# jinkyu032/TPDM

Measured on NVIDIA B200. Metric: images/sec/box, SD3-M 1024^2 TPDM sampling, higher is better.
Workload: dtype bf16

## Files before the change

tpdm_b200/csrc/gemm2_tcgen05.cu:

```cuda
#include <cuda_bf16.h>

#include "common.cuh"
#include "gemm_epilogue.cuh"
#include "host.h"

namespace tpdm {

namespace {

constexpr int BM = 128;
constexpr int BN2 = 256;
#ifndef TPDM_GEMM2_BK
#define TPDM_GEMM2_BK 64
#endif
constexpr int BK = TPDM_GEMM2_BK;
constexpr int kSub = BK / 64;
constexpr int kStages2 = BK == 64 ? 5 : 3;
constexpr int kEpiWarps2 = 8;
constexpr int kThreads2 = 64 + 32 * kEpiWarps2;
constexpr int kABytes2 = BM * BK * 2;
constexpr int kBBytes2 = (BN2 / 2) * BK * 2;
constexpr int kStageBytes2 = kABytes2 + kBBytes2;
constexpr int kRing2 = kStages2 * kStageBytes2;
constexpr int kEpi2 = kEpiWarps2 * 32 * kStagePad * 4 + kEpiWarps2 * 2 * (BN2 / 2) * 4;
constexpr int kBarOff2 = kRing2 + kEpi2;
constexpr int kSmem2 = kBarOff2 + 256 + 1024;

#ifdef TPDM_GEMM_TRACE
__device__ long long g_gemm_trace[4096];
__device__ int g_gemm_trace_n;
#endif

struct Gemm2Params {
  GemmOp op[2];
  int n_ops;
  int tiles0, total_tiles;
  const int* skip;
  const int* bmask;
  int bslots;
};

struct PairCoord {
  int g, b, mtp, nt;
};

__device__ __forceinline__ PairCoord decode_pair(const Gemm2Params& P, int tile) {
  PairCoord t;
  t.g = (P.n_ops > 1 && tile >= P.tiles0) ? 1 : 0;
  const int local = tile - (t.g ? P.tiles0 : 0);
  const GemmOp& G = P.op[t.g];
  const int tiles_mp = (G.rows_per_batch + 2 * BM - 1) / (2 * BM);
  const int m_idx = local / G.tiles_n;
  t.nt = local - m_idx * G.tiles_n;
  t.b = m_idx / tiles_mp;
  t.mtp = m_idx - t.b * tiles_mp;
  return t;
}

__device__ __forceinline__ uint32_t cluster_ctarank() {
  uint32_t r;
  asm volatile("mov.u32 %0, %%cluster_ctarank;" : "=r"(r));
  return r;
}
__device__ __forceinline__ void cluster_sync_all() {
  asm volatile("barrier.cluster.arrive.release.aligned;\n\tbarrier.cluster.wait.acquire.aligned;\n" ::: "memory");
}
__device__ __forceinline__ uint32_t map_to_cta(const void* p, uint32_t rank) {
  uint32_t r;
  asm volatile("mapa.shared::cluster.u32 %0, %1, %2;" : "=r"(r) : "r"(smem_u32(p)), "r"(rank));
  return r;
}
__device__ __forceinline__ void mbar_arrive_expect_tx_cluster(uint32_t cluster_addr, uint32_t bytes) {
  asm volatile("mbarrier.arrive.expect_tx.shared::cluster.b64 _, [%0], %1;" ::"r"(cluster_addr), "r"(bytes) : "memory");
}
__device__ __forceinline__ void mbar_arrive_cluster(uint32_t cluster_addr) {
  asm volatile("mbarrier.arrive.shared::cluster.b64 _, [%0];" ::"r"(cluster_addr) : "memory");
}
__device__ __forceinline__ void tma2_load_3d(void* smem_dst, const CUtensorMap* m, uint32_t bar_cluster_addr, int c0, int c1, int c2) {
  asm volatile(
      "cp.async.bulk.tensor.3d.cta_group::2.shared::cluster.global.mbarrier::complete_tx::bytes [%0], [%1, {%3, %4, %5}], [%2];\n" ::"r"(
          smem_u32(smem_dst)),
      "l"(reinterpret_cast<uint64_t>(m)), "r"(bar_cluster_addr), "r"(c0), "r"(c1), "r"(c2)
      : "memory");
}
__device__ __forceinline__ void tma2_load_2d(void* smem_dst, const CUtensorMap* m, uint32_t bar_cluster_addr, int c0, int c1) {
  asm volatile(
      "cp.async.bulk.tensor.2d.cta_group::2.shared::cluster.global.mbarrier::complete_tx::bytes [%0], [%1, {%3, %4}], [%2];\n" ::"r"(
          smem_u32(smem_dst)),
      "l"(reinterpret_cast<uint64_t>(m)), "r"(bar_cluster_addr), "r"(c0), "r"(c1)
      : "memory");
}
__device__ __forceinline__ void umma2_ss(uint32_t d_tmem, uint64_t a_desc, uint64_t b_desc, uint32_t idesc, uint32_t accumulate) {
  asm volatile(
      "{\n\t.reg .pred p;\n\t"
      "setp.ne.b32 p, %4, 0;\n\t"
      "tcgen05.mma.cta_group::2.kind::f16 [%0], %1, %2, %3, p;\n\t}\n" ::"r"(d_tmem),
      "l"(a_desc), "l"(b_desc), "r"(idesc), "r"(accumulate)
      : "memory");
}
__device__ __forceinline__ void umma2_ss_elect(uint32_t d_tmem, uint64_t a_desc, uint64_t b_desc, uint32_t idesc, uint32_t accumulate) {
  asm volatile(
      "{\n\t.reg .pred p, e;\n\t"
      "elect.sync _|e, 0xffffffff;\n\t"
      "setp.ne.b32 p, %4, 0;\n\t"
      "@e tcgen05.mma.cta_group::2.kind::f16 [%0], %1, %2, %3, p;\n\t}\n" ::"r"(d_tmem),
      "l"(a_desc), "l"(b_desc), "r"(idesc), "r"(accumulate)
      : "memory");
}
__device__ __forceinline__ void umma2_commit_multicast_elect(uint64_t* bar) {
  asm volatile(
      "{\n\t.reg .pred e;\n\t"
      "elect.sync _|e, 0xffffffff;\n\t"
      "@e tcgen05.commit.cta_group::2.mbarrier::arrive::one.shared::cluster.multicast::cluster.b64 [%0], %1;\n\t}\n" ::"r"(smem_u32(bar)),
      "h"(static_cast<uint16_t>(3))
      : "memory");
}
__device__ __forceinline__ void umma2_commit_multicast(uint64_t* bar) {
  asm volatile("tcgen05.commit.cta_group::2.mbarrier::arrive::one.shared::cluster.multicast::cluster.b64 [%0], %1;\n" ::"r"(smem_u32(bar)),
               "h"(static_cast<uint16_t>(3))
               : "memory");
}

__global__ void __cluster_dims__(2, 1, 1) __launch_bounds__(kThreads2, 1) gemm2_bf16_tcgen05_kernel(const __grid_constant__ Gemm2Params P) {
  pdl_launch_dependents();
  extern __shared__ uint8_t smem_raw[];
  uint8_t* smem = reinterpret_cast<uint8_t*>((reinterpret_cast<uintptr_t>(smem_raw) + 1023) & ~uintptr_t(1023));
  float* epi_stage = reinterpret_cast<float*>(smem + kRing2);
  uint64_t* full_bar = reinterpret_cast<uint64_t*>(smem + kBarOff2);
  uint64_t* empty_bar = full_bar + kStages2;
  uint64_t* tmem_full = empty_bar + kStages2;
  uint64_t* tmem_empty = tmem_full + 2;
  uint32_t* tmem_slot = reinterpret_cast<uint32_t*>(tmem_empty + 2);

  const int warp = threadIdx.x >> 5;
  const int lane = threadIdx.x & 31;
  const uint32_t rank = cluster_ctarank();
  const int cluster_id = blockIdx.x >> 1, num_clusters = gridDim.x >> 1;

  if (warp == 0 && lane == 0) {
    for (int i = 0; i < P.n_ops; ++i) {
      tma_prefetch_desc(&P.op[i].tmA);
      tma_prefetch_desc(&P.op[i].tmB2);
    }
  }
  if (warp == 1 && lane == 0) {
    for (int i = 0; i < kStages2; ++i) {
      mbar_init(&full_bar[i], 2);
      mbar_init(&empty_bar[i], 1);
    }
    for (int i = 0; i < 2; ++i) {
      mbar_init(&tmem_full[i], 1);
      mbar_init(&tmem_empty[i], 2 * kEpiWarps2);
    }
    fence_barrier_init();
  }
  pdl_wait();
  if (P.skip != nullptr && *P.skip != 0) return;
  if (warp == 2) {
    asm volatile("tcgen05.alloc.cta_group::2.sync.aligned.shared::cta.b32 [%0], 512;\n" ::"r"(smem_u32(tmem_slot)) : "memory");
    asm volatile("tcgen05.relinquish_alloc_permit.cta_group::2.sync.aligned;\n" ::: "memory");
  }
  tc_fence_before();
  cluster_sync_all();
  tc_fence_after();
  const uint32_t tmem_base = *tmem_slot;

  if (warp == 0) {
    if (lane == 0) {
      int stage = 0;
      uint32_t phase = 0;
      for (int tile = cluster_id; tile < P.total_tiles; tile += num_clusters) {
        const PairCoord tc = decode_pair(P, tile);
        if (P.bmask != nullptr && P.bmask[tc.b % P.bslots] == 0) continue;
        const GemmOp& G = P.op[tc.g];
        const int nkb = (G.K + BK - 1) / BK;
        const int m0 = tc.mtp * 2 * BM + static_cast<int>(rank) * BM;
        const int nb0 = tc.nt * BN2 + static_cast<int>(rank) * (BN2 / 2);
        for (int kb = 0; kb < nkb; ++kb) {
          mbar_wait_backoff(&empty_bar[stage], phase ^ 1);
          uint8_t* sA = smem + stage * kStageBytes2;
          uint8_t* sB = sA + kABytes2;
          const uint32_t leader_full = map_to_cta(&full_bar[stage], 0);
          mbar_arrive_expect_tx_cluster(leader_full, kStageBytes2);
#pragma unroll
          for (int h = 0; h < kSub; ++h) {
            tma2_load_3d(sA + h * (BM * 128), &G.tmA, leader_full, kb * BK + h * 64, m0, tc.b);
            tma2_load_2d(sB + h * ((BN2 / 2) * 128), &G.tmB2, leader_full, kb * BK + h * 64, nb0);
          }
          if (++stage == kStages2) {
            stage = 0;
            phase ^= 1;
          }
        }
      }
    }
  } else if (warp == 1) {
    if (rank == 0) {
      constexpr uint32_t idesc = make_idesc_bf16(2 * BM, BN2);
      int stage = 0;
      uint32_t phase = 0;
      int acc = 0;
      uint32_t acc_phase = 0;
      for (int tile = cluster_id; tile < P.total_tiles; tile += num_clusters) {
        const PairCoord tc = decode_pair(P, tile);
        if (P.bmask != nullptr && P.bmask[tc.b % P.bslots] == 0) continue;
        const GemmOp& G = P.op[tc.g];
        const int nkb = (G.K + BK - 1) / BK;
#ifdef TPDM_GEMM_TRACE
        const bool tr = cluster_id == 0 && lane == 0;
        long long tq0 = 0;
        if (tr) tq0 = clock64();
#endif
        mbar_wait(&tmem_empty[acc], acc_phase ^ 1);
        tc_fence_after();
#ifdef TPDM_GEMM_TRACE
        if (tr && g_gemm_trace_n + 4 <= 4096) {
          g_gemm_trace[g_gemm_trace_n++] = -1;
          g_gemm_trace[g_gemm_trace_n++] = tq0;
          g_gemm_trace[g_gemm_trace_n++] = clock64();
          g_gemm_trace[g_gemm_trace_n++] = nkb;
        }
#endif
        const uint32_t d_tmem = tmem_base + acc * BN2;
        for (int kb = 0; kb < nkb; ++kb) {
#ifdef TPDM_GEMM_TRACE
          long long t0 = 0, t1 = 0;
          if (tr) t0 = clock64();
#endif
          mbar_wait(&full_bar[stage], phase);
          tc_fence_after();
#ifdef TPDM_GEMM_TRACE
          if (tr) t1 = clock64();
#endif
          {
            const uint32_t a_base = smem_u32(smem + stage * kStageBytes2);
            const uint32_t b_base = a_base + kABytes2;
            const uint64_t adesc0 = make_smem_desc_sw128(a_base, 16, 1024), bdesc0 = make_smem_desc_sw128(b_base, 16, 1024);
#pragma unroll
            for (int k = 0; k < BK / 16; ++k) {
              const uint32_t ao = ((k / 4) * (BM * 128) + (k % 4) * 32) >> 4, bo = ((k / 4) * ((BN2 / 2) * 128) + (k % 4) * 32) >> 4;
              umma2_ss_elect(d_tmem, adesc0 + ao, bdesc0 + bo, idesc, (kb | k) != 0 ? 1u : 0u);
            }
            umma2_commit_multicast_elect(&empty_bar[stage]);
            if (kb == nkb - 1) umma2_commit_multicast_elect(&tmem_full[acc]);
          }
#ifdef TPDM_GEMM_TRACE
          if (tr && g_gemm_trace_n + 3 <= 4096) {
            g_gemm_trace[g_gemm_trace_n++] = t0;
            g_gemm_trace[g_gemm_trace_n++] = t1;
            g_gemm_trace[g_gemm_trace_n++] = clock64();
          }
#endif
          __syncwarp();
          if (++stage == kStages2) {
            stage = 0;
            phase ^= 1;
          }
        }
        if (++acc == 2) {
          acc = 0;
          acc_phase ^= 1;
        }
      }
    }
  } else {
    const int q = warp & 3;
    const int hh = (warp - 2) >> 2;
    float* st = epi_stage + (warp - 2) * 32 * kStagePad;
    float* sbias = epi_stage + kEpiWarps2 * 32 * kStagePad + (warp - 2) * 2 * (BN2 / 2);
    int acc = 0;
    uint32_t acc_phase = 0;
    for (int tile = cluster_id; tile < P.total_tiles; tile += num_clusters) {
      const PairCoord tc = decode_pair(P, tile);
        if (P.bmask != nullptr && P.bmask[tc.b % P.bslots] == 0) continue;
      const GemmOp& G = P.op[tc.g];
      const int n0 = tc.nt * BN2;
      const int row_base = tc.mtp * 2 * BM + static_cast<int>(rank) * BM + q * 32;
      gemm_epilogue_tile<BN2>(
          G, tc.b, row_base, n0, tmem_base + (static_cast<uint32_t>(q * 32) << 16) + acc * BN2, st, sbias, lane, hh * (BN2 / 64), (hh + 1) * (BN2 / 64),
          [&]() { mbar_wait_backoff(&tmem_full[acc], acc_phase); },
          [&]() {
            if (lane == 0) mbar_arrive_cluster(map_to_cta(&tmem_empty[acc], 0));
          });
      if (++acc == 2) {
        acc = 0;
        acc_phase ^= 1;
      }
    }
  }

  __syncwarp();
  tc_fence_before();
  cluster_sync_all();
  if (warp == 2) asm volatile("tcgen05.dealloc.cta_group::2.sync.aligned.b32 %0, 512;\n" ::"r"(tmem_base) : "memory");
}

}

#ifdef TPDM_GEMM_TRACE
extern "C" int tpdm_gemm_trace_read(long long* host, int* n, int reset) {
  int cnt = 0;
  if (cudaMemcpyFromSymbol(&cnt, g_gemm_trace_n, sizeof(int)) != cudaSuccess) return -1;
  if (cudaMemcpyFromSymbol(host, g_gemm_trace, sizeof(long long) * 4096) != cudaSuccess) return -1;
  *n = cnt;
  if (reset) {
    cnt = 0;
    cudaMemcpyToSymbol(g_gemm_trace_n, &cnt, sizeof(int));
  }
  return 0;
}
#endif

int gemm2_launch(const GemmOp* ops, int n_ops, cudaStream_t stream) {
  TPDM_CHECK(n_ops >= 1 && n_ops <= 2, TPDM_ERR_ARG, "gemm2_launch: 1 or 2 ops per launch");
  Gemm2Params P;
  P.n_ops = n_ops;
  P.total_tiles = 0;
  P.tiles0 = 0;
  P.skip = skip_flag();
  P.bmask = batch_mask();
  P.bslots = batch_mask_slots();
  double flops = 0;
  for (int i = 0; i < n_ops; ++i) {
    TPDM_CHECK(ops[i].conv == 0 && ops[i].block_n == 256, TPDM_ERR_ARG, "gemm2_launch: plain GEMMs with 256-wide N tiles only");
    P.op[i] = ops[i];
    const int tiles_mp = (ops[i].rows_per_batch + 2 * BM - 1) / (2 * BM);
    const int t = ops[i].batch * tiles_mp * ops[i].tiles_n;
    if (i == 0) P.tiles0 = t;
    P.total_tiles += t;
    flops += 2.0 * ops[i].batch * ops[i].rows_per_batch * static_cast<double>(ops[i].N) * ops[i].K;
  }
  if (n_ops == 1) P.op[1] = ops[0];
  static bool attr_set = false;
  if (!attr_set) {
    TPDM_CUDA_OK(cudaFuncSetAttribute(gemm2_bf16_tcgen05_kernel, cudaFuncAttributeMaxDynamicSharedMemorySize, kSmem2));
    attr_set = true;
  }
  const int max_clusters = num_sms() / 2;
  const int clusters = P.total_tiles < max_clusters ? P.total_tiles : max_clusters;
  prof_begin(0, flops, stream);
  TPDM_CUDA_OK(launch_pdl(gemm2_bf16_tcgen05_kernel, dim3(2 * clusters), dim3(kThreads2), kSmem2, stream, P));
  prof_end(stream);
  count_launch();
  TPDM_CUDA_OK(cudaGetLastError());
  return 0;
}

}
```

tpdm_b200/csrc/gemm_epilogue.cuh:

```cuda
#pragma once
#include <cuda_bf16.h>

#include "common.cuh"
#include "host.h"

namespace tpdm {

constexpr int kStagePad = 36;

template <int BN, typename WaitFn, typename ReleaseFn>
__device__ __forceinline__ void gemm_epilogue_tile(const GemmOp& G, int batch_idx, int row_base, int n0, uint32_t tmem_acc, float* st,
                                                   float* sbias, int lane, int c_begin, int c_end, WaitFn wait_accumulator,
                                                   ReleaseFn release_accumulator) {
  int n_chunks = (G.N - n0 + 31) / 32;
  n_chunks = n_chunks > c_end ? c_end : n_chunks;
  const int ncol = (c_end - c_begin) * 32;
  if (n_chunks <= c_begin) {
    wait_accumulator();
    tc_fence_after();
    tc_fence_before();
    __syncwarp();
    release_accumulator();
    return;
  }
      int rows = G.rows_per_batch - row_base;
      rows = rows > 32 ? 32 : rows;
      const bool f32_out = G.epi == EPI_BIAS_F32 || G.epi == EPI_GATE_RESIDUAL;
      const bool add_bf16 = G.epi == EPI_BIAS_ADD_BF16;
      const bool resid = G.epi == EPI_GATE_RESIDUAL;
      const int vec = 4;
      const int cg = lane % 8;
      const int r_in = lane / 8;
      const float* gate_row = resid ? G.gate + static_cast<long long>(batch_idx) * G.gate_stride : nullptr;
      const long long tile_o0 = static_cast<long long>(batch_idx) * G.out_batch_stride + static_cast<long long>(row_base) * G.ldo + n0;

      auto load_resv = [&](int c, float4 (&rv)[8]) {
        const int col = n0 + c * 32 + cg * 4;
        if (col < G.N) {
          const float* o = reinterpret_cast<const float*>(G.out) + tile_o0 + c * 32 + cg * 4;
#pragma unroll
          for (int it = 0; it < 8; ++it) {
            const int r = it * 4 + r_in;
            rv[it] = r < rows ? *reinterpret_cast<const float4*>(o + static_cast<long long>(r) * G.ldo) : make_float4(0.f, 0.f, 0.f, 0.f);
          }
        }
      };
      for (int k = lane * 4; k < ncol; k += 128) {
        const int col = n0 + c_begin * 32 + k;
        float4 b4 = make_float4(0.f, 0.f, 0.f, 0.f), g4 = b4;
        if (col < G.N) {
          if (G.bias) b4 = *reinterpret_cast<const float4*>(G.bias + col);
          if (resid) g4 = *reinterpret_cast<const float4*>(gate_row + col);
        }
        *reinterpret_cast<float4*>(sbias + k) = b4;
        *reinterpret_cast<float4*>(sbias + ncol + k) = g4;
      }
      __syncwarp();
      float4 resv_a[8], resv_b[8];
      if (resid) {
        if (lane < rows) {
          const float* o = reinterpret_cast<const float*>(G.out) + tile_o0 + static_cast<long long>(lane) * G.ldo;
          for (int c = c_begin + 1; c < n_chunks; ++c) asm volatile("prefetch.global.L2 [%0];" ::"l"(o + c * 32));
        }
        load_resv(c_begin, resv_a);
      }
      wait_accumulator();
      tc_fence_after();

      auto process_chunk = [&](int c, const float4 (&resv)[8]) {
        const int col = n0 + c * 32 + cg * vec;
        const bool col_ok = col < G.N && rows > 0;
        const long long o0 = tile_o0 + c * 32 + cg * vec;
        float bias[4], gate[4];
        {
          const float* sb = sbias + (c - c_begin) * 32 + cg * 4;
          const float4 b0 = *reinterpret_cast<const float4*>(sb);
          bias[0] = b0.x; bias[1] = b0.y; bias[2] = b0.z; bias[3] = b0.w;
          const float4 g4 = *reinterpret_cast<const float4*>(sb + ncol);
          gate[0] = g4.x; gate[1] = g4.y; gate[2] = g4.z; gate[3] = g4.w;
        }
        uint32_t v[32];
        tmem_ld_32x32(tmem_acc + c * 32, v);
        tmem_wait_ld();
        if (c == n_chunks - 1) {
          tc_fence_before();
          __syncwarp();
          release_accumulator();
        }
        if (!f32_out) {
          if (lane < rows && n0 + c * 32 < G.N) {
            const bool gelu = G.epi == EPI_BIAS_GELU_BF16;
            const float* sb = sbias + (c - c_begin) * 32;
            __nv_bfloat16* o = reinterpret_cast<__nv_bfloat16*>(G.out) + tile_o0 + c * 32 + static_cast<long long>(lane) * G.ldo;
#pragma unroll
            for (int q = 0; q < 4; ++q) {
              const float4 b0 = *reinterpret_cast<const float4*>(sb + 8 * q);
              const float4 b1 = *reinterpret_cast<const float4*>(sb + 8 * q + 4);
              float y[8] = {__uint_as_float(v[8 * q]) + b0.x,     __uint_as_float(v[8 * q + 1]) + b0.y,
                            __uint_as_float(v[8 * q + 2]) + b0.z, __uint_as_float(v[8 * q + 3]) + b0.w,
                            __uint_as_float(v[8 * q + 4]) + b1.x, __uint_as_float(v[8 * q + 5]) + b1.y,
                            __uint_as_float(v[8 * q + 6]) + b1.z, __uint_as_float(v[8 * q + 7]) + b1.w};
              if (gelu) {
#pragma unroll
                for (int e = 0; e < 8; ++e) y[e] = gelu_tanh(y[e]);
              }
              if (add_bf16 && n0 + c * 32 + 8 * q < G.N) {
                const uint4 a = *reinterpret_cast<const uint4*>(reinterpret_cast<const __nv_bfloat16*>(G.res) + (o - reinterpret_cast<__nv_bfloat16*>(G.out)) + 8 * q);
                y[0] += __uint_as_float(a.x << 16); y[1] += __uint_as_float(a.x & 0xffff0000u);
                y[2] += __uint_as_float(a.y << 16); y[3] += __uint_as_float(a.y & 0xffff0000u);
                y[4] += __uint_as_float(a.z << 16); y[5] += __uint_as_float(a.z & 0xffff0000u);
                y[6] += __uint_as_float(a.w << 16); y[7] += __uint_as_float(a.w & 0xffff0000u);
              }
              uint4 w;
              w.x = pack_bf16x2(y[0], y[1]);
              w.y = pack_bf16x2(y[2], y[3]);
              w.z = pack_bf16x2(y[4], y[5]);
              w.w = pack_bf16x2(y[6], y[7]);
              if (n0 + c * 32 + 8 * q < G.N) *reinterpret_cast<uint4*>(o + 8 * q) = w;
            }
          }
          return;
        }
#pragma unroll
        for (int j = 0; j < 8; ++j)
          *reinterpret_cast<uint4*>(st + lane * kStagePad + 4 * j) = make_uint4(v[4 * j], v[4 * j + 1], v[4 * j + 2], v[4 * j + 3]);
        __syncwarp();
        if (col_ok) {
          {
            float* o = reinterpret_cast<float*>(G.out) + o0;
#pragma unroll
            for (int it = 0; it < 8; ++it) {
              const int r = it * 4 + r_in;
              if (r < rows) {
                const float4 x = *reinterpret_cast<const float4*>(st + r * kStagePad + cg * 4);
                float4 y = make_float4(x.x + bias[0], x.y + bias[1], x.z + bias[2], x.w + bias[3]);
                if (resid)
                  y = make_float4(resv[it].x + gate[0] * y.x, resv[it].y + gate[1] * y.y, resv[it].z + gate[2] * y.z,
                                  resv[it].w + gate[3] * y.w);
                *reinterpret_cast<float4*>(o + static_cast<long long>(r) * G.ldo) = y;
              }
            }
          }
        }
        __syncwarp();
      };

      for (int c = c_begin; c < n_chunks; c += 2) {
        if (resid && c + 1 < n_chunks) load_resv(c + 1, resv_b);
        process_chunk(c, resv_a);
        if (c + 1 < n_chunks) {
          if (resid && c + 2 < n_chunks) load_resv(c + 2, resv_a);
          process_chunk(c + 1, resv_b);
        }
      }
}

}
```

Before: 2.303.

## Pack M blocks across batch boundaries in 2-CTA GEMM pair tiles

Tile decoding for the cluster-pair GEMM now counts 128-row M blocks globally across batches and pairs consecutive blocks, instead of padding each batch to a multiple of 256 rows. Each CTA gets its own batch index and row offset, and a CTA whose half is masked or out of range skips its A load and epilogue while still loading B for the shared MMA. This removes wasted pair tiles when rows per batch is not a multiple of 256, and lets partially masked pairs do half the loads. It adds per-rank expect-tx byte accounting and more decode logic per tile.

```diff
diff --git a/tpdm_b200/csrc/gemm2_tcgen05.cu b/tpdm_b200/csrc/gemm2_tcgen05.cu
--- a/tpdm_b200/csrc/gemm2_tcgen05.cu
+++ b/tpdm_b200/csrc/gemm2_tcgen05.cu
@@ -41,20 +41,42 @@
 };
 
 struct PairCoord {
-  int g, b, mtp, nt;
+  int g, nt;
+  int b, m0;
+  bool active;
+  bool idle;
 };
 
-__device__ __forceinline__ PairCoord decode_pair(const Gemm2Params& P, int tile) {
+__device__ __forceinline__ PairCoord decode_pair(const Gemm2Params& P, int tile, uint32_t rank) {
   PairCoord t;
   t.g = (P.n_ops > 1 && tile >= P.tiles0) ? 1 : 0;
   const int local = tile - (t.g ? P.tiles0 : 0);
   const GemmOp& G = P.op[t.g];
-  const int tiles_mp = (G.rows_per_batch + 2 * BM - 1) / (2 * BM);
   const int m_idx = local / G.tiles_n;
   t.nt = local - m_idx * G.tiles_n;
-  t.b = m_idx / tiles_mp;
-  t.mtp = m_idx - t.b * tiles_mp;
+  const int blocks = G.batch * G.tiles_m_per_batch;
+  bool act[2];
+#pragma unroll
+  for (int h = 0; h < 2; ++h) {
+    const int blk = 2 * m_idx + h;
+    const int b = blk / G.tiles_m_per_batch;
+    act[h] = blk < blocks && (P.bmask == nullptr || P.bmask[b % P.bslots] != 0);
+    if (h == static_cast<int>(rank)) {
+      t.b = b;
+      t.m0 = (blk - b * G.tiles_m_per_batch) * BM;
+    }
+  }
+  t.active = rank != 0 ? act[1] : act[0];
+  t.idle = !act[0] && !act[1];
   return t;
+}
+
+template <typename Fn>
+__device__ __forceinline__ void for_each_tile(const Gemm2Params& P, int c, int nc, uint32_t rank, Fn&& fn) {
+  for (int tile = c; tile < P.total_tiles; tile += nc) {
+    const PairCoord tc = decode_pair(P, tile, rank);
+    if (!tc.idle) fn(tc);
+  }
 }
 
 __device__ __forceinline__ uint32_t cluster_ctarank() {
@@ -169,22 +191,20 @@
     if (lane == 0) {
       int stage = 0;
       uint32_t phase = 0;
-      for (int tile = cluster_id; tile < P.total_tiles; tile += num_clusters) {
-        const PairCoord tc = decode_pair(P, tile);
-        if (P.bmask != nullptr && P.bmask[tc.b % P.bslots] == 0) continue;
+      for_each_tile(P, cluster_id, num_clusters, rank, [&](const PairCoord& tc) {
         const GemmOp& G = P.op[tc.g];
+        const int nb0 = tc.nt * BN2 + static_cast<int>(rank) * (BN2 / 2);
+        const uint32_t bytes = tc.active ? kStageBytes2 : kBBytes2;
         const int nkb = (G.K + BK - 1) / BK;
-        const int m0 = tc.mtp * 2 * BM + static_cast<int>(rank) * BM;
-        const int nb0 = tc.nt * BN2 + static_cast<int>(rank) * (BN2 / 2);
         for (int kb = 0; kb < nkb; ++kb) {
           mbar_wait_backoff(&empty_bar[stage], phase ^ 1);
           uint8_t* sA = smem + stage * kStageBytes2;
           uint8_t* sB = sA + kABytes2;
           const uint32_t leader_full = map_to_cta(&full_bar[stage], 0);
-          mbar_arrive_expect_tx_cluster(leader_full, kStageBytes2);
+          mbar_arrive_expect_tx_cluster(leader_full, bytes);
 #pragma unroll
           for (int h = 0; h < kSub; ++h) {
-            tma2_load_3d(sA + h * (BM * 128), &G.tmA, leader_full, kb * BK + h * 64, m0, tc.b);
+            if (tc.active) tma2_load_3d(sA + h * (BM * 128), &G.tmA, leader_full, kb * BK + h * 64, tc.m0, tc.b);
             tma2_load_2d(sB + h * ((BN2 / 2) * 128), &G.tmB2, leader_full, kb * BK + h * 64, nb0);
           }
           if (++stage == kStages2) {
@@ -192,7 +212,7 @@
             phase ^= 1;
           }
         }
-      }
+      });
     }
   } else if (warp == 1) {
     if (rank == 0) {
@@ -201,9 +221,7 @@
       uint32_t phase = 0;
       int acc = 0;
       uint32_t acc_phase = 0;
-      for (int tile = cluster_id; tile < P.total_tiles; tile += num_clusters) {
-        const PairCoord tc = decode_pair(P, tile);
-        if (P.bmask != nullptr && P.bmask[tc.b % P.bslots] == 0) continue;
+      for_each_tile(P, cluster_id, num_clusters, rank, [&](const PairCoord& tc) {
         const GemmOp& G = P.op[tc.g];
         const int nkb = (G.K + BK - 1) / BK;
 #ifdef TPDM_GEMM_TRACE
@@ -261,32 +279,35 @@
           acc = 0;
           acc_phase ^= 1;
         }
-      }
+      });
     }
   } else {
     const int q = warp & 3;
-    const int hh = (warp - 2) >> 2;
-    float* st = epi_stage + (warp - 2) * 32 * kStagePad;
-    float* sbias = epi_stage + kEpiWarps2 * 32 * kStagePad + (warp - 2) * 2 * (BN2 / 2);
+    const int ew = warp - 2;
+    const int hh = ew >> 2;
+    const int c_begin = hh * (BN2 / 64), c_end = (hh + 1) * (BN2 / 64);
+    float* st = epi_stage + ew * 32 * kStagePad;
+    float* sbias = epi_stage + kEpiWarps2 * 32 * kStagePad + ew * 2 * (BN2 / 2);
     int acc = 0;
     uint32_t acc_phase = 0;
-    for (int tile = cluster_id; tile < P.total_tiles; tile += num_clusters) {
-      const PairCoord tc = decode_pair(P, tile);
-        if (P.bmask != nullptr && P.bmask[tc.b % P.bslots] == 0) continue;
+    for_each_tile(P, cluster_id, num_clusters, rank, [&](const PairCoord& tc) {
       const GemmOp& G = P.op[tc.g];
       const int n0 = tc.nt * BN2;
-      const int row_base = tc.mtp * 2 * BM + static_cast<int>(rank) * BM + q * 32;
-      gemm_epilogue_tile<BN2>(
-          G, tc.b, row_base, n0, tmem_base + (static_cast<uint32_t>(q * 32) << 16) + acc * BN2, st, sbias, lane, hh * (BN2 / 64), (hh + 1) * (BN2 / 64),
-          [&]() { mbar_wait_backoff(&tmem_full[acc], acc_phase); },
-          [&]() {
-            if (lane == 0) mbar_arrive_cluster(map_to_cta(&tmem_empty[acc], 0));
-          });
+      const int row_base = tc.m0 + q * 32;
+      const uint32_t tmem_acc = tmem_base + (static_cast<uint32_t>(q * 32) << 16) + acc * BN2;
+      auto wait = [&]() { mbar_wait_backoff(&tmem_full[acc], acc_phase); };
+      auto release = [&]() {
+        if (lane == 0) mbar_arrive_cluster(map_to_cta(&tmem_empty[acc], 0));
+      };
+      if (!tc.active || row_base >= G.rows_per_batch)
+        gemm_epilogue_skip(wait, release);
+      else
+        gemm_epilogue_tile<BN2>(G, tc.b, row_base, n0, tmem_acc, st, sbias, lane, c_begin, c_end, wait, release);
       if (++acc == 2) {
         acc = 0;
         acc_phase ^= 1;
       }
-    }
+    });
   }
 
   __syncwarp();
@@ -324,8 +345,8 @@
   for (int i = 0; i < n_ops; ++i) {
     TPDM_CHECK(ops[i].conv == 0 && ops[i].block_n == 256, TPDM_ERR_ARG, "gemm2_launch: plain GEMMs with 256-wide N tiles only");
     P.op[i] = ops[i];
-    const int tiles_mp = (ops[i].rows_per_batch + 2 * BM - 1) / (2 * BM);
-    const int t = ops[i].batch * tiles_mp * ops[i].tiles_n;
+    const int blocks = ops[i].batch * ops[i].tiles_m_per_batch;
+    const int t = (blocks + 1) / 2 * ops[i].tiles_n;
     if (i == 0) P.tiles0 = t;
     P.total_tiles += t;
     flops += 2.0 * ops[i].batch * ops[i].rows_per_batch * static_cast<double>(ops[i].N) * ops[i].K;
diff --git a/tpdm_b200/csrc/gemm_epilogue.cuh b/tpdm_b200/csrc/gemm_epilogue.cuh
--- a/tpdm_b200/csrc/gemm_epilogue.cuh
+++ b/tpdm_b200/csrc/gemm_epilogue.cuh
@@ -8,6 +8,15 @@
 
 constexpr int kStagePad = 36;
 
+template <typename WaitFn, typename ReleaseFn>
+__device__ __forceinline__ void gemm_epilogue_skip(WaitFn wait_accumulator, ReleaseFn release_accumulator) {
+  wait_accumulator();
+  tc_fence_after();
+  tc_fence_before();
+  __syncwarp();
+  release_accumulator();
+}
+
 template <int BN, typename WaitFn, typename ReleaseFn>
 __device__ __forceinline__ void gemm_epilogue_tile(const GemmOp& G, int batch_idx, int row_base, int n0, uint32_t tmem_acc, float* st,
                                                    float* sbias, int lane, int c_begin, int c_end, WaitFn wait_accumulator,
@@ -16,11 +25,7 @@
   n_chunks = n_chunks > c_end ? c_end : n_chunks;
   const int ncol = (c_end - c_begin) * 32;
   if (n_chunks <= c_begin) {
-    wait_accumulator();
-    tc_fence_after();
-    tc_fence_before();
-    __syncwarp();
-    release_accumulator();
+    gemm_epilogue_skip(wait_accumulator, release_accumulator);
     return;
   }
       int rows = G.rows_per_batch - row_base;
```

After: 2.314, median of 6. About the same (+0.5%).
